# wpeebles/gangealing

Measured on NVIDIA H100. Metric: gangealing_train_images_per_sec_256, higher is better.
Workload: dtype f32

## Files before the change

### __graft_entry__.py

```python
import os
import sys

ROOT = os.path.dirname(os.path.abspath(__file__))
if ROOT not in sys.path:
    sys.path.insert(0, ROOT)


def build():
    from gangealing_b200 import build as gg_build
    lib = gg_build.build()
    from gangealing_b200 import _lib
    _lib.load()
    import gangealing_b200.op
    if os.path.isdir("/root/reference"):
        try:
            from oracle import build_ref
            build_ref.build()
        except Exception as exc:
            print("oracle/_ref not built: %s" % exc, file=sys.stderr)
    return lib


def smoke():
    import torch
# ... 37 lines not shown
          so.upfirdn2d_ref(x[:, :3], k, up=2, pad=(2, 1)), 1e-5)
    close("fused_leaky_relu", op.fused_leaky_relu(x.to(dev), b.to(dev)), so.fused_leaky_relu_ref(x, b), 1e-6)

    for dt, tol in ((torch.float32, 1e-4), (torch.bfloat16, 2e-2)):
        n, c = 2, 64
        raw = torch.randn(n, c, 17, 17, generator=g).to(dt).float()
        d, s_next = torch.rand(n, c, generator=g) + 0.5, torch.randn(n, c, generator=g) + 1
        nz = torch.randn(n, 1, 16, 16, generator=g)
        bb = torch.randn(c, generator=g)
        lo = [t.clone().requires_grad_(True) for t in (raw, d, s_next)]
        xs_o = so.blur_noise_bias_act_ref(lo[0], k, (1, 1), nz, nw, bb, row_scale=lo[1]) * lo[2][:, :, None, None]
        go = torch.randn(xs_o.shape, generator=g).to(dt).float()
        gr_o = torch.autograd.grad(xs_o, lo, go)
        lg = [raw.to(dev).to(dt).contiguous(memory_format=CL).requires_grad_(True), d.to(dev).requires_grad_(True),
              s_next.to(dev).requires_grad_(True)]
        xs, _ = fused_tail(lg[0], lg[1], lg[2], None, None, nz.to(dev), nw.to(dev), bb.to(dev), None, kernel=k.to(dev), pad=(1, 1))
        gr = torch.autograd.grad(xs, lg, go.to(dev).to(dt).contiguous(memory_format=CL))
        close("channels-last blur tail -> next conv input (%s)" % str(dt)[6:], xs, xs_o, tol)
        close("  its one-pass backward: d raw / d demod / d style (%s)" % str(dt)[6:], torch.cat([t.flatten().float().cpu() for t in gr]),
              torch.cat([t.flatten() for t in gr_o]), tol)
        raw2 = torch.randn(n, c, 16, 16, generator=g).to(dt).float()
        wm = torch.randn(n, 3, c, generator=g) / 8
        rb, skip = torch.randn(3, generator=g), torch.randn(n, 3, 16, 16, generator=g)
        o_ = so.noise_bias_act_ref(raw2 * d[:, :, None, None], nz, nw, bb)
        rgb_o = torch.einsum("noc,nchw->nohw", wm, o_) + rb.reshape(1, 3, 1, 1) + skip
        _, rgb = fused_tail(raw2.to(dev).to(dt).contiguous(memory_format=CL), d.to(dev), None, wm.to(dev), skip.to(dev), nz.to(dev),
                            nw.to(dev), bb.to(dev), rb.to(dev))
        close("channels-last conv tail + to-RGB in one pass (%s)" % str(dt)[6:], rgb, rgb_o, tol)

    w = [torch.randn(1, 128, 64, 3, 3, generator=g), torch.randn(1, 256, 128, 3, 3, generator=g)]
    st = [torch.randn(3, 64, generator=g), torch.randn(3, 128, generator=g)]
    dm = style_path.all_demod([t.to(dev) for t in w], [t.to(dev) for t in st], [0.04, 0.03])
    for wi, si, sc, di in zip(w, st, (0.04, 0.03), dm):
        want = torch.rsqrt(((sc * wi) * si.reshape(3, 1, -1, 1, 1)).pow(2).sum([2, 3, 4]) + 1e-8)
        close("wgmma demodulation GEMM (O=%d, I=%d)" % (wi.shape[1], wi.shape[2]), di, want, 1e-5)

    img = torch.rand(2, 3, 64, 64, generator=g) * 2 - 1
    theta = torch.tensor([[[0.7, 0.2, 0.05], [-0.2, 0.6, -0.1]], [[1.6, 0.0, 0.0], [0.0, 1.5, 0.1]]])
    out, grid, _ = S.stn_sample_affine(img.to(dev), theta.to(dev), (64, 64), 3.5, 0.0, "border")
    grid_o = osmp.affine_grid_ref(theta, (2, 3, 64, 64))
    close("one-pass similarity sampling: grid", grid, grid_o, 1e-5)
    close("one-pass similarity sampling: antialiased warp", out, osmp.mipmap_warp_ref(img, grid_o, 3.5, 0.0, "border"), 2e-3)
    low = 0.03 * torch.randn(2, 8, 8, 2, generator=g)
    mask = torch.randn(2, 576, 8, 8, generator=g)
    ident = osmp.affine_grid_ref(torch.eye(2, 3)[None], (1, 1, 64, 64))
    out, flow, delta, _ = S.stn_sample_flow(img.to(dev), low.to(dev), mask.to(dev), ident.to(dev), theta.to(dev), None, 8, 3.5, 0.0,
                                            "reflection")
    delta_o, flow_o = of.flow_compose_ref(low, mask, ident, theta, None, 8)
    close("one-pass flow sampling: composed flow", flow, flow_o, 1e-5)
    close("one-pass flow sampling: antialiased warp", out, osmp.mipmap_warp_ref(img, flow_o, 3.5, 0.0, "reflection"), 2e-3)
    close("BilinearDownsample (tent gather)", S.bilinear_downsample(img.to(dev), 2, *[t.to(dev) for t in _tent(3)]),
# ... 75 lines not shown
```

### gangealing_b200/_lib.py

```python
import ctypes
import os

import torch

_HERE = os.path.dirname(os.path.abspath(__file__))
LIB_PATH = os.path.join(_HERE, "libgg_b200.so")

GG_F32, GG_F16, GG_BF16 = 0, 1, 2
PAD_MODES = {"zeros": 0, "border": 1, "reflection": 2}

_c = ctypes
_P, _I, _L, _F = _c.c_void_p, _c.c_int, _c.c_int64, _c.c_float

SIGNATURES = {
    "gg_version": (_I, []),
    "gg_last_error": (_c.c_char_p, []),
    "gg_sm_count": (_I, []),
    "gg_fused_bias_act": (_I, [_P, _P, _P, _P, _I, _I, _I, _F, _F, _L, _L, _L, _P]),
    "gg_noise_bias_act": (_I, [_P, _P, _P, _P, _P, _P, _I, _F, _F, _L, _L, _L, _P]),
    "gg_channel_scale_workspace": (_L, [_L, _L]),
    "gg_channel_scale": (_I, [_P, _P, _P, _P, _P, _P, _I, _L, _L, _P]),
    "gg_bias_act_backward_workspace": (_L, [_L, _L, _L]),
    "gg_bias_act_backward": (_I, [_P, _P, _P, _P, _P, _I, _F, _F, _L, _L, _L, _P]),
    "gg_upfirdn2d": (_I, [_P, _P, _P, _I, _L] + [_I] * 12 + [_P]),
    "gg_blur_noise_bias_act": (_I, [_P] * 7 + [_I, _L, _L] + [_I] * 9 + [_F, _F, _P]),
    "gg_mipmap_pyramid_elems": (_L, [_L, _I, _I, _I]),
    "gg_mipmap_build": (_I, [_P, _P, _I, _L, _I, _I, _I, _P]),
    "gg_mipmap_build_backward": (_I, [_P, _P, _L, _I, _I, _I, _P]),
    "gg_mipmap_warp_forward": (_I, [_P] * 5 + [_I, _L] + [_I] * 6 + [_F, _F, _I, _P]),
    "gg_warp_sample_indices": (_I, [_P, _P, _L, _I, _I, _I, _I, _F, _F, _I, _P]),
    "gg_stn_sample_forward": (_I, [_P] * 11 + [_I, _I, _L] + [_I] * 9 + [_F, _F, _I, _P]),
    "gg_modconv_wsq": (_I, [_P, _P, _I, _I, _I, _P]),
    "gg_modconv_demod": (_I, [_P, _P, _P, _F, _F, _I, _I, _I, _P]),
    "gg_modconv_demod_batched": (_I, [_I, _P, _P, _P, _P, _P, _P, _F, _I, _P]),
    "gg_modconv_modulate": (_I, [_P, _P, _P, _P, _F, _I, _I, _I, _I, _I, _P]),
    "gg_noise_bias_act_nhwc": (_I, [_P] * 6 + [_I, _F, _F, _L, _I, _L, _P]),
    "gg_nhwc_rowwise_workspace": (_L, [_L, _I, _L]),
    "gg_channel_scale_nhwc": (_I, [_P] * 6 + [_I, _L, _I, _L, _P]),
    "gg_bias_act_backward_nhwc": (_I, [_P] * 5 + [_I, _F, _F, _L, _I, _L, _P]),
    "gg_blur_nhwc_workspace": (_L, [_I, _L] + [_I] * 9),
    "gg_blur_nhwc": (_I, [_P] * 12 + [_I, _L] + [_I] * 12 + [_F, _F, _P]),
    "gg_styled_tail_nhwc": (_I, [_P] * 12 + [_I, _I, _F, _F, _L, _I, _L, _P]),
    "gg_styled_tail_backward_workspace": (_L, [_I, _L, _I, _L]),
    "gg_styled_tail_backward_nhwc": (_I, [_P] * 12 + [_I, _F, _F, _L, _I, _L, _L, _P]),
    "gg_tent_downsample_forward": (_I, [_P] * 4 + [_L, _I, _I, _I, _I, _P]),
    "gg_tent_downsample_backward": (_I, [_P] * 4 + [_L, _I, _I, _I, _I, _P]),
    "gg_feature_distance_workspace": (_L, [_L, _I, _L]),
    "gg_feature_distance_forward": (_I, [_P] * 5 + [_I, _L, _I, _L, _F, _P]),
    "gg_feature_distance_backward": (_I, [_P] * 6 + [_I, _L, _I, _L, _F, _P]),
    "gg_bias_relu_pool_nhwc_forward": (_I, [_P, _P, _P, _P, _I, _L, _I, _I, _I, _P]),
    "gg_bias_relu_pool_nhwc_backward": (_I, [_P, _P, _P, _P, _I, _L, _I, _I, _I, _P]),
    "gg_to_rgb_nhwc_workspace": (_L, [_L, _I, _L]),
    "gg_to_rgb_nhwc_forward": (_I, [_P] * 5 + [_L, _I, _L, _P]),
    "gg_to_rgb_nhwc_backward": (_I, [_P] * 6 + [_L, _I, _L, _P]),
    "gg_nn_argmin_workspace": (_L, [_L, _L]),
    "gg_nn_argmin": (_I, [_P, _P, _P, _P, _L, _L, _I, _P]),
    "gg_splat2d_lookup_forward": (_I, [_P] * 8 + [_L, _L, _I, _I, _I, _I, _I, _F, _F, _I, _P]),
    "gg_scale_cast_multi": (_I, [_P, _P, _P, _I, _I, _P]),
    "gg_adam_ema_step": (_I, [_P, _P, _P, _I, _I, _P, _c.c_double, _c.c_double, _c.c_double, _c.c_double, _P]),
    "gg_tv_loss_workspace": (_L, [_L, _I, _I]),
    "gg_tv_loss_forward": (_I, [_P, _P, _P, _L, _I, _I, _P]),
    "gg_tv_loss_backward": (_I, [_P, _P, _P, _L, _I, _I, _P]),
    "gg_splat2d_workspace": (_L, [_L, _I, _I, _I]),
    "gg_splat2d_forward": (_I, [_P] * 6 + [_L, _L, _I, _I, _I, _I, _P]),
    "gg_flow_compose_forward": (_I, [_P] * 7 + [_L, _I, _I, _I, _P]),
    "gg_flow_compose_backward": (_I, [_P] * 10 + [_L, _I, _I, _I, _P]),
    "gg_mipmap_warp_backward": (_I, [_P] * 7 + [_I, _L] + [_I] * 6 + [_F, _F, _I, _P]),
# ... 143 lines not shown
```

### gangealing_b200/csrc/styled.cu

```cuda
#include "common.cuh"
#include "nhwc_reduce.cuh"

namespace gg {
namespace {

constexpr int kT = 256;
constexpr int kGroup = 8;
constexpr int kPix = 4;

struct TailFwdParams {
  const void* raw; void* out; void* xs; float* rgb; const float* skip;
  const float* noise; const float* noise_weight; const float* bias; const float* demod; const float* s_next;
  const float* wm; const float* rgb_bias;
  float alpha, gain;
  int act;
  int C;
  int64_t hw;
  int chunk, chunks_per_sample;
};

template <typename T, bool FAST>
__global__ void __launch_bounds__(kT, 2)
styled_tail_nhwc_kernel(const TailFwdParams p) {
  constexpr int V = ChanVec<T>::V;
  constexpr int Q = V / 4;
  extern __shared__ __align__(16) float cst[];
  const int C = p.C;
  const int nvec = C / V, J = nvec / kGroup;
  const int64_t n = blockIdx.x / p.chunks_per_sample;
  const int ck = blockIdx.x - n * p.chunks_per_sample;
  const int64_t p0 = static_cast<int64_t>(ck) * p.chunk, p1 = min(p0 + p.chunk, p.hw);
// ... 19 lines not shown
  const int l = threadIdx.x & (kGroup - 1), grp = threadIdx.x / kGroup;
  const unsigned gmask = 0xffu << (threadIdx.x & 24);
  const int hw = static_cast<int>(p.hw);
  const T* raw = static_cast<const T*>(p.raw) + n * hw * C;
  T* out = p.out ? static_cast<T*>(p.out) + n * hw * C : nullptr;
  T* xs = p.xs ? static_cast<T*>(p.xs) + n * hw * C : nullptr;
  const float* noise_n = p.noise ? p.noise + n * hw : nullptr;
  const int q0 = static_cast<int>(p0), q1 = static_cast<int>(p1);
  constexpr int kStride = (kT / kGroup) * kPix;
  auto pixel = [&](int pb_, int u) { return min(pb_ + u, q1 - 1); };
  uint4 xn[kPix];
  int pb = q0 + grp * kPix;
  if (pb < q1) {
#pragma unroll
    for (int u = 0; u < kPix; ++u) xn[u] = ldg_stream16(raw + static_cast<unsigned>(pixel(pb, u) * C + l * V));
  }
  for (; pb < q1; pb += kStride) {
    float nz[kPix];
    unsigned po[kPix];
#pragma unroll
    for (int u = 0; u < kPix; ++u) {
      const int px = pixel(pb, u);
      po[u] = static_cast<unsigned>(px) * static_cast<unsigned>(C);
      nz[u] = noise_n ? nw * __ldg(noise_n + px) : 0.f;
    }
    float acc[kPix][3];
#pragma unroll
    for (int u = 0; u < kPix; ++u) acc[u][0] = acc[u][1] = acc[u][2] = 0.f;
    for (int j = 0; j < J; ++j) {
      const int v = l + kGroup * j;
      uint4 xr[kPix];
#pragma unroll
      for (int u = 0; u < kPix; ++u) xr[u] = xn[u];
      {
        const bool wrap = (j + 1 == J);
        const int pbn = wrap ? pb + kStride : pb;
        const int vn = wrap ? l : v + kGroup;
        if (pbn < q1) {
#pragma unroll
          for (int u = 0; u < kPix; ++u) xn[u] = ldg_stream16(raw + static_cast<unsigned>(pixel(pbn, u) * C + vn * V));
        }
      }
      float d[V], b[V], s[V], w0[V], w1[V], w2[V];
#pragma unroll
      for (int q = 0; q < Q; ++q) {
        const float4 dv = c4[q * nvec + v], bv = c4[c4_plane + q * nvec + v], sv = c4[2 * c4_plane + q * nvec + v];
        d[4 * q] = dv.x; d[4 * q + 1] = dv.y; d[4 * q + 2] = dv.z; d[4 * q + 3] = dv.w;
        b[4 * q] = bv.x; b[4 * q + 1] = bv.y; b[4 * q + 2] = bv.z; b[4 * q + 3] = bv.w;
        s[4 * q] = sv.x; s[4 * q + 1] = sv.y; s[4 * q + 2] = sv.z; s[4 * q + 3] = sv.w;
        if (p.rgb) {
          const float4 a0 = c4[3 * c4_plane + q * nvec + v], a1 = c4[4 * c4_plane + q * nvec + v], a2 = c4[5 * c4_plane + q * nvec + v];
          w0[4 * q] = a0.x; w0[4 * q + 1] = a0.y; w0[4 * q + 2] = a0.z; w0[4 * q + 3] = a0.w;
          w1[4 * q] = a1.x; w1[4 * q + 1] = a1.y; w1[4 * q + 2] = a1.z; w1[4 * q + 3] = a1.w;
          w2[4 * q] = a2.x; w2[4 * q + 1] = a2.y; w2[4 * q + 2] = a2.z; w2[4 * q + 3] = a2.w;
        }
      }
#pragma unroll
      for (int u = 0; u < kPix; ++u) {
        float x[V], o[V], o2[V];
        ChanVec<T>::unpack(xr[u], x);
#pragma unroll
        for (int k = 0; k < V; ++k) {
          float t = fmaf(x[k], d[k], b[k] + nz[u]);
          t = fast ? fmaxf(t, t * neg) : (t > 0.f ? t : t * neg) * p.gain;
          o[k] = t;
          o2[k] = t * s[k];
        }
        if (p.rgb) {
#pragma unroll
          for (int k = 0; k < V; ++k) {
            acc[u][0] = fmaf(w0[k], o[k], acc[u][0]);
            acc[u][1] = fmaf(w1[k], o[k], acc[u][1]);
            acc[u][2] = fmaf(w2[k], o[k], acc[u][2]);
          }
        }
        if (pb + u < q1) {
          const unsigned off = po[u] + static_cast<unsigned>(v * V);
          if (out) stg_stream16(out + off, ChanVec<T>::pack(o));
          if (xs) stg_stream16(xs + off, ChanVec<T>::pack(o2));
        }
      }
    }
    if (p.rgb) {
#pragma unroll
      for (int m = kGroup / 2; m >= 1; m >>= 1)
#pragma unroll
        for (int u = 0; u < kPix; ++u)
#pragma unroll
          for (int o = 0; o < 3; ++o) acc[u][o] += __shfl_xor_sync(gmask, acc[u][o], m);
      if (l < 3) {
        const int o = l;
        const float rb = p.rgb_bias ? __ldg(p.rgb_bias + o) : 0.f;
        const int64_t off = (n * 3 + o) * p.hw + pb;
#pragma unroll
        for (int u = 0; u < kPix; ++u)
          if (pb + u < q1) {
            const float r = (o == 0 ? acc[u][0] : o == 1 ? acc[u][1] : acc[u][2]) + rb;
            p.rgb[off + u] = r + (p.skip ? __ldg(p.skip + off + u) : 0.f);
          }
      }
    }
  }
}

struct TailBwdParams {
  void* g_raw; float* partial;
  const void* g_xs; const void* out; const void* raw;
  const float* s_next; const float* demod; const float* g_rgb; const float* wm;
  float alpha, gain;
  int C;
  int64_t hw;
  int chunk, chunks_per_sample;
  int r_ds, r_dd, r_gw, n_red;
};

template <typename T>
__global__ void __launch_bounds__(kT, 2)
styled_tail_bwd_nhwc_kernel(const TailBwdParams p) {
  constexpr int V = ChanVec<T>::V;
  constexpr int U = (V == 4) ? 4 : 2;
  extern __shared__ float red[];
  const int C = p.C, cv = C / V;
  const int64_t n = blockIdx.x / p.chunks_per_sample;
  const int ck = blockIdx.x - n * p.chunks_per_sample;
  const int64_t p0 = static_cast<int64_t>(ck) * p.chunk, p1 = min(p0 + p.chunk, p.hw);
  const int lanes_p = kT / cv > 0 ? kT / cv : 1;
  const int cq = threadIdx.x % cv, pl = threadIdx.x / cv;
  float a_ds[V], a_dd[V], a_g0[V], a_g1[V], a_g2[V];
#pragma unroll
  for (int k = 0; k < V; ++k) a_ds[k] = a_dd[k] = a_g0[k] = a_g1[k] = a_g2[k] = 0.f;
  const T* gxs = static_cast<const T*>(p.g_xs);
  const T* outp = static_cast<const T*>(p.out);
  const T* rawp = static_cast<const T*>(p.raw);
  T* graw = static_cast<T*>(p.g_raw);
  if (pl < lanes_p) {
    float sv[V], dv[V], w0[V], w1[V], w2[V];
#pragma unroll
    for (int k = 0; k < V; ++k) {
      const int c = cq * V + k;
      sv[k] = p.s_next ? __ldg(p.s_next + n * C + c) : 1.f;
      dv[k] = p.demod ? __ldg(p.demod + n * C + c) : 1.f;
      w0[k] = p.g_rgb ? __ldg(p.wm + (n * 3 + 0) * C + c) : 0.f;
      w1[k] = p.g_rgb ? __ldg(p.wm + (n * 3 + 1) * C + c) : 0.f;
      w2[k] = p.g_rgb ? __ldg(p.wm + (n * 3 + 2) * C + c) : 0.f;
    }
    const float* g0 = p.g_rgb ? p.g_rgb + n * 3 * p.hw : nullptr;
    const uint4 zero = make_uint4(0u, 0u, 0u, 0u);
    auto body = [&](int64_t off, const uint4 gr, const uint4 orw, const uint4 rr, float s0, float s1, float s2) {
      float g[V], o[V], r[V], gt[V];
      ChanVec<T>::unpack(gr, g);
      ChanVec<T>::unpack(orw, o);
      ChanVec<T>::unpack(rr, r);
#pragma unroll
      for (int k = 0; k < V; ++k) {
        float go = g[k] * sv[k];
        if (p.g_rgb) go = fmaf(w2[k], s2, fmaf(w1[k], s1, fmaf(w0[k], s0, go)));
        const float t = (o[k] > 0.f ? go : go * p.alpha) * p.gain;
        a_ds[k] = fmaf(g[k], o[k], a_ds[k]);
        a_dd[k] = fmaf(t, r[k], a_dd[k]);
        a_g0[k] = fmaf(s0, o[k], a_g0[k]);
        a_g1[k] = fmaf(s1, o[k], a_g1[k]);
        a_g2[k] = fmaf(s2, o[k], a_g2[k]);
        gt[k] = t * dv[k];
      }
      *reinterpret_cast<uint4*>(graw + off) = ChanVec<T>::pack(gt);
    };
    int64_t pp = p0 + pl;
    for (; pp + (U - 1) * lanes_p < p1; pp += U * lanes_p) {
      uint4 gr[U], orw[U], rr[U];
      float s[U][3];
      int64_t off[U];
#pragma unroll
      for (int u = 0; u < U; ++u) {
        const int64_t pu = pp + u * lanes_p;
        off[u] = ((n * p.hw + pu) * cv + cq) * V;
        orw[u] = ldg_stream16(outp + off[u]);
        gr[u] = gxs ? ldg_stream16(gxs + off[u]) : zero;
      }
#pragma unroll
      for (int u = 0; u < U; ++u) {
        const int64_t pu = pp + u * lanes_p;
        rr[u] = rawp ? ldg_stream16(rawp + off[u]) : zero;
        s[u][0] = g0 ? __ldg(g0 + pu) : 0.f;
        s[u][1] = g0 ? __ldg(g0 + p.hw + pu) : 0.f;
        s[u][2] = g0 ? __ldg(g0 + 2 * p.hw + pu) : 0.f;
      }
#pragma unroll
      for (int u = 0; u < U; ++u) body(off[u], gr[u], orw[u], rr[u], s[u][0], s[u][1], s[u][2]);
    }
    for (; pp < p1; pp += lanes_p) {
      const int64_t off = ((n * p.hw + pp) * cv + cq) * V;
      body(off, gxs ? ldg_stream16(gxs + off) : zero, ldg_stream16(outp + off), rawp ? ldg_stream16(rawp + off) : zero,
           g0 ? __ldg(g0 + pp) : 0.f, g0 ? __ldg(g0 + p.hw + pp) : 0.f, g0 ? __ldg(g0 + 2 * p.hw + pp) : 0.f);
    }
  }
  if (p.partial && p.n_red > 0) {
    const int R = p.n_red;
    if (pl < lanes_p) {
      float* row = red + static_cast<int64_t>(pl) * R * C + cq * V;
#pragma unroll
      for (int k = 0; k < V; ++k) {
        if (p.r_ds >= 0) row[p.r_ds * C + k] = a_ds[k];
        if (p.r_dd >= 0) row[p.r_dd * C + k] = a_dd[k];
        if (p.r_gw >= 0) { row[p.r_gw * C + k] = a_g0[k]; row[(p.r_gw + 1) * C + k] = a_g1[k]; row[(p.r_gw + 2) * C + k] = a_g2[k]; }
      }
    }
    __syncthreads();
    for (int i = threadIdx.x; i < R * C; i += kT) {
      float t = 0.f;
      for (int q = 0; q < lanes_p; ++q) t += red[static_cast<int64_t>(q) * R * C + i];
      p.partial[static_cast<int64_t>(blockIdx.x) * R * C + i] = t;
    }
  }
}

// ... 50 lines not shown
  const size_t smem = static_cast<size_t>(6) * C * sizeof(float);
  auto st = static_cast<cudaStream_t>(stream);
  const bool fast = p.gain > 0.f && ((p.act == 3 && p.alpha >= 0.f && p.alpha <= 1.f) || p.act == 1);
  const unsigned g = static_cast<unsigned>(grid);
  if (dtype == GG_F32) {
    if (fast) styled_tail_nhwc_kernel<float, true><<<g, kT, smem, st>>>(p);
    else styled_tail_nhwc_kernel<float, false><<<g, kT, smem, st>>>(p);
  } else {
    if (fast) styled_tail_nhwc_kernel<__nv_bfloat16, true><<<g, kT, smem, st>>>(p);
    else styled_tail_nhwc_kernel<__nv_bfloat16, false><<<g, kT, smem, st>>>(p);
  }
  GG_CHECK_LAUNCH("styled_tail_nhwc launch");
  return GG_OK;
}

int64_t gg_styled_tail_backward_workspace(int dtype, int64_t N, int C, int64_t HW) {
  if (N <= 0 || C <= 0 || HW <= 0) return 0;
  const int V = dtype == GG_BF16 ? 8 : 4;
  if (C % V != 0) return 0;
  const int64_t chunk = bwd_chunk(N, C / V, HW);
  return N * ((HW + chunk - 1) / chunk) * 5 * C * static_cast<int64_t>(sizeof(float));
}

int gg_styled_tail_backward_nhwc(void* g_raw, float* d_s_next, float* d_demod, float* d_wm, void* workspace,
                                 const void* g_xs, const float* g_rgb, const void* out_saved, const void* raw,
                                 const float* s_next, const float* demod, const float* wm, int dtype, float alpha,
                                 float scale, int64_t N, int C, int64_t HW, int64_t reduce_pitch, void* stream) {
  if (N < 0 || C < 0 || HW < 0) return fail(GG_ERR_BAD_ARG, "styled_tail_backward_nhwc: negative size");
  if (dtype != GG_F32 && dtype != GG_BF16) return fail(GG_ERR_UNSUPPORTED, "styled_tail_backward_nhwc: dtype %d not supported", dtype);
  if (N * HW * C == 0) return GG_OK;
  const int V = dtype == GG_BF16 ? 8 : 4;
  if (C % V != 0 || C / V > kT) return fail(GG_ERR_UNSUPPORTED, "styled_tail_backward_nhwc: C must be a multiple of %d, <= %d", V, V * kT);
  if (!g_raw || !out_saved || (!g_xs && !g_rgb)) return fail(GG_ERR_BAD_ARG, "styled_tail_backward_nhwc: null tensor");
  if (g_xs && !s_next) return fail(GG_ERR_BAD_ARG, "styled_tail_backward_nhwc: g_xs needs s_next");
  if (g_rgb && !wm) return fail(GG_ERR_BAD_ARG, "styled_tail_backward_nhwc: g_rgb needs wm");
  if (d_s_next && !g_xs) return fail(GG_ERR_BAD_ARG, "styled_tail_backward_nhwc: d_s_next needs g_xs");
  if (d_demod && !raw) return fail(GG_ERR_BAD_ARG, "styled_tail_backward_nhwc: d_demod needs raw");
  if (d_wm && !g_rgb) return fail(GG_ERR_BAD_ARG, "styled_tail_backward_nhwc: d_wm needs g_rgb");
  if ((d_s_next || d_demod || d_wm) && !workspace) return fail(GG_ERR_BAD_ARG, "styled_tail_backward_nhwc: reductions need a workspace");
  const int cv = C / V;
  const int64_t chunk64 = bwd_chunk(N, cv, HW);
  if (chunk64 > 0x7fffffffLL) return fail(GG_ERR_BAD_ARG, "styled_tail_backward_nhwc: plane too large");
  const int K = static_cast<int>((HW + chunk64 - 1) / chunk64);
  const int64_t grid = N * K;
  if (grid > 0x7fffffffLL) return fail(GG_ERR_BAD_ARG, "styled_tail_backward_nhwc: too many CTAs");
  TailBwdParams p;
  p.g_raw = g_raw; p.partial = static_cast<float*>(workspace); p.g_xs = g_xs; p.out = out_saved;
  p.raw = d_demod ? raw : nullptr; p.s_next = s_next; p.demod = demod; p.g_rgb = g_rgb; p.wm = wm;
  p.alpha = alpha; p.gain = scale; p.C = C; p.hw = HW; p.chunk = static_cast<int>(chunk64); p.chunks_per_sample = K;
  int r = 0;
  p.r_ds = d_s_next ? r++ : -1;
  p.r_dd = d_demod ? r++ : -1;
  p.r_gw = d_wm ? r : -1;
  if (d_wm) r += 3;
  p.n_red = r;
  const int lanes_p = kT / cv > 0 ? kT / cv : 1;
  const size_t smem = static_cast<size_t>(lanes_p) * (r > 0 ? r : 1) * C * sizeof(float);
  auto st = static_cast<cudaStream_t>(stream);
  if (smem > 48 * 1024) {
    static DeviceOnce configured;
    if (configured.needed()) {
      cudaError_t e = cudaFuncSetAttribute(styled_tail_bwd_nhwc_kernel<float>, cudaFuncAttributeMaxDynamicSharedMemorySize, 100 * 1024);
      if (e == cudaSuccess)
        e = cudaFuncSetAttribute(styled_tail_bwd_nhwc_kernel<__nv_bfloat16>, cudaFuncAttributeMaxDynamicSharedMemorySize, 100 * 1024);
      if (e != cudaSuccess) return cuda_fail(e, "styled_tail_backward_nhwc smem opt-in");
      configured.done();
    }
    if (smem > 100 * 1024) return fail(GG_ERR_UNSUPPORTED, "styled_tail_backward_nhwc: C too large for the reduction stage");
  }
  if (dtype == GG_F32) styled_tail_bwd_nhwc_kernel<float><<<static_cast<unsigned>(grid), kT, smem, st>>>(p);
  else styled_tail_bwd_nhwc_kernel<__nv_bfloat16><<<static_cast<unsigned>(grid), kT, smem, st>>>(p);
  GG_CHECK_LAUNCH("styled_tail_backward_nhwc launch");
  if (r > 0) {
    float* first = d_s_next ? d_s_next : (d_demod ? d_demod : d_wm);
    const bool packed = (!d_s_next || d_s_next == first + static_cast<int64_t>(p.r_ds) * C) &&
                        (!d_demod || d_demod == first + static_cast<int64_t>(p.r_dd) * C) &&
                        (!d_wm || d_wm == first + static_cast<int64_t>(p.r_gw) * C) && reduce_pitch == r * C;
    if (packed) {
      nhwc_finish_kernel<<<static_cast<unsigned>(N * ((r * C + 31) / 32)), dim3(32, 32), 0, st>>>(
          first, static_cast<const float*>(workspace), N, K, r * C, r * C);
    } else {
      auto finish_row = [&](float* dst, int row, int rows_n) {
        nhwc_finish_kernel<<<static_cast<unsigned>(N * ((rows_n * C + 31) / 32)), dim3(32, 32), 0, st>>>(
            dst, static_cast<const float*>(workspace) + static_cast<int64_t>(row) * C, N, K, rows_n * C, r * C);
      };
      if (reduce_pitch != C && reduce_pitch != 0 && reduce_pitch != r * C)
        return fail(GG_ERR_BAD_ARG, "styled_tail_backward_nhwc: reduce_pitch must be C (separate dense outputs) or r*C (packed block)");
      if (d_s_next) finish_row(d_s_next, p.r_ds, 1);
      if (d_demod) finish_row(d_demod, p.r_dd, 1);
      if (d_wm) finish_row(d_wm, p.r_gw, 3);
    }
    GG_CHECK_LAUNCH("styled_tail_backward_nhwc finish launch");
  }
  return GG_OK;
}

}
```

### gangealing_b200/op/nhwc.py

```python
import torch

from .. import _lib

CL = torch.channels_last

TIMING = None


def elementwise_ok(t):
    return _lib.is_nhwc(t) and t.shape[1] % _lib.nhwc_vec(t) == 0


def rowwise_ok(t):
    return elementwise_ok(t) and t.shape[1] // _lib.nhwc_vec(t) <= 256


def blur_ok(t, kh, kw, up=(1, 1), down=(1, 1)):
    return (_lib.is_nhwc(t) and t.shape[1] % (8 * _lib.nhwc_vec(t)) == 0 and kh <= 4 and kw <= 4
            and up == (1, 1) and down == (1, 1))


def _f32(t, numel=None):
    if t is None:
        return None
# ... 99 lines not shown


def styled_tail(raw, noise, noise_weight, bias, demod, s_next, wm, rgb_bias, skip, want_out, negative_slope, gain, act=3):
    n, c, h, w = raw.shape
    out = torch.empty_like(raw) if want_out else None
    xs = torch.empty_like(raw) if s_next is not None else None
    rgb = torch.empty((n, 3, h, w), dtype=torch.float32, device=raw.device) if wm is not None else None
    sk = None
    if skip is not None and rgb is not None:
        sk = skip.detach()
        if sk.dtype != torch.float32 or not sk.is_contiguous():
            sk = sk.float().contiguous()
        if sk.shape != rgb.shape:
            raise RuntimeError("styled_tail: skip must be (N, 3, H, W)")
    rc = _lib.load().gg_styled_tail_nhwc(_lib.ptr(out), _lib.ptr(xs), _lib.ptr(rgb), raw.data_ptr(),
                                         _lib.ptr(noise_plane(noise, n, h, w)), _lib.ptr(_f32(noise_weight, 1)),
                                         _lib.ptr(_f32(bias, c)), _lib.ptr(_f32(demod, n * c)), _lib.ptr(_f32(s_next, n * c)),
                                         _lib.ptr(_f32(wm, n * 3 * c)), _lib.ptr(_f32(rgb_bias, 3)), _lib.ptr(sk),
                                         _lib.dtype_code(raw), act, negative_slope, gain, n, c, h * w, _lib.stream())
    _lib.check(rc, "gg_styled_tail_nhwc")
    return out, xs, rgb


def styled_tail_backward(g_xs, g_rgb, out_saved, raw, s_next, demod, wm, want_ds, want_dd, want_dwm, negative_slope, gain):
    n, c, h, w = out_saved.shape
    lib = _lib.load()
    dev = out_saved.device
    g_raw = torch.empty_like(out_saved)
    want_ds = want_ds and g_xs is not None
    want_dd = want_dd and raw is not None
    want_dwm = want_dwm and g_rgb is not None
    rows = int(want_ds) + int(want_dd) + 3 * int(want_dwm)
    block = torch.empty((n, rows, c), dtype=torch.float32, device=dev) if rows else None
    r = 0
    d_s = d_d = d_w = None
    if want_ds:
        d_s = block[:, r]; r += 1
    if want_dd:
        d_d = block[:, r]; r += 1
    if want_dwm:
        d_w = block[:, r:r + 3]
    code = _lib.dtype_code(out_saved)
    ws = None
    if rows:
        ws = torch.empty(max(1, lib.gg_styled_tail_backward_workspace(code, n, c, h * w) // 4), dtype=torch.float32, device=dev)
    rc = lib.gg_styled_tail_backward_nhwc(g_raw.data_ptr(), _lib.ptr(d_s), _lib.ptr(d_d), _lib.ptr(d_w), _lib.ptr(ws),
                                          _lib.ptr(g_xs), _lib.ptr(g_rgb), out_saved.data_ptr(),
                                          _lib.ptr(raw if want_dd else None),
                                          _lib.ptr(_f32(s_next, n * c)), _lib.ptr(_f32(demod, n * c)), _lib.ptr(_f32(wm, n * 3 * c)),
                                          code, negative_slope, gain, n, c, h * w, rows * c, _lib.stream())
    _lib.check(rc, "gg_styled_tail_backward_nhwc")
    return g_raw, d_s, d_d, d_w
```

### gangealing_b200/op/styled_fused.py

```python
import torch
from torch.autograd import Function
from torch.autograd.function import once_differentiable

from .. import _lib
from . import conv2d_gradfix, nhwc, style_path
from .modconv import channel_scale, shared_conv_weight
from .upfirdn2d import grad_pad, upfirdn2d

CL = torch.channels_last


class _FusedTail(Function):

    @staticmethod
    def forward(ctx, raw, demod, s_next, wm, skip, noise, noise_weight, bias, rgb_bias, kernel, pad, negative_slope, gain):
        _lib.require_cuda(raw, demod, s_next, wm, skip, noise)
        needs = ctx.needs_input_grad
        save = needs[0] or needs[1] or needs[2] or needs[3]
        if kernel is None:
            out, xs, rgb = nhwc.styled_tail(raw, noise, noise_weight, bias, demod, s_next, wm, rgb_bias, skip, save,
                                            negative_slope, gain)
        else:
            if wm is not None:
                raise RuntimeError("fused tail: the blur (up-sampling) layers carry no to-RGB branch")
            pad4 = (pad[0], pad[1], pad[0], pad[1])
            out, xs, _ = nhwc.blur(raw, kernel, pad4, mode=1, noise=noise, noise_weight=noise_weight, bias=bias,
                                   row_scale=demod, scale2=s_next, want_out=save or s_next is None,
                                   want_out2=s_next is not None, negative_slope=negative_slope, gain=gain)
            rgb = None
        ctx.cfg = (kernel is not None, pad, negative_slope, gain, tuple(raw.shape))
        if save:
            ctx.save_for_backward(raw if (needs[1] and demod is not None) else None, out,
                                  demod.detach() if demod is not None else None,
                                  s_next.detach() if s_next is not None else None,
                                  wm.detach() if wm is not None else None, kernel)
        if skip is not None and rgb is None:
            raise RuntimeError("fused tail: skip without a to-RGB branch")
        return xs, rgb

    @staticmethod
    @once_differentiable
    def backward(ctx, g_xs, g_rgb):
        raw, out, demod, s_next, wm, kernel = ctx.saved_tensors
        is_blur, pad, negative_slope, gain, raw_shape = ctx.cfg
        need_raw, need_d, need_s, need_w, need_skip = ctx.needs_input_grad[:5]
        if g_xs is not None:
            g_xs = g_xs.contiguous(memory_format=CL)
            if g_xs.dtype != out.dtype:
                g_xs = g_xs.to(out.dtype)
        if g_rgb is not None:
            g_rgb = g_rgb.float().contiguous()
        g_raw = d_s = d_d = d_w = None
        if g_xs is None and g_rgb is None:
            return (None,) * 13
        if not is_blur:
            g_raw, d_s, d_d, d_w = nhwc.styled_tail_backward(
                g_xs, g_rgb, out, raw, s_next, demod, wm, need_s, need_d and demod is not None, need_w,
                negative_slope, gain)
        else:
            g_t, d_s, _, _ = nhwc.styled_tail_backward(g_xs, None, out, None, s_next, None, None, need_s, False, False,
                                                       negative_slope, gain)
            kh, kw = kernel.shape
            pad4 = (pad[0], pad[1], pad[0], pad[1])
            gp = grad_pad(raw_shape[2], raw_shape[3], out.shape[2], out.shape[3], kh, kw, (1, 1), (1, 1), pad4)
            want_dot = need_d and demod is not None
            g_raw, _, d_d = nhwc.blur(g_t, _lib.flipped_filter(kernel), gp, mode=2, row_scale=demod, mul=raw if want_dot else None,
                                      want_dot=want_dot)
            if tuple(g_raw.shape) != raw_shape:
                raise RuntimeError("fused tail backward: adjoint produced %s, expected %s" % (tuple(g_raw.shape), raw_shape))
        return (g_raw if need_raw else None, d_d if need_d else None, d_s if need_s else None, d_w if need_w else None,
                g_rgb if need_skip else None, None, None, None, None, None, None, None, None)


def fused_tail(raw, demod, s_next, wm, skip, noise, noise_weight, bias, rgb_bias, kernel=None, pad=None, negative_slope=0.2,
               gain=2 ** 0.5):
    return _FusedTail.apply(raw, demod, s_next, wm, skip, noise, noise_weight, bias, rgb_bias, kernel, pad, negative_slope, gain)


def fusable(generator, latent, act_dtype):
    if not latent.is_cuda or getattr(generator, "num_fp16_res", 0) != 0 and not generator.run_fp32:
        return False
# ... 58 lines not shown
```

### include/gg_b200.h

```cpp
#ifndef GG_B200_H_
#define GG_B200_H_

#include <stdint.h>

#ifdef __cplusplus
extern "C" {
#endif

#define GG_API __attribute__((visibility("default")))

enum { GG_F32 = 0, GG_F16 = 1, GG_BF16 = 2, GG_F64 = 3 };

enum {
  GG_OK = 0,
  GG_ERR_BAD_ARG = -1,
  GG_ERR_UNSUPPORTED = -2,
  GG_ERR_CUDA = -3
};

enum { GG_PAD_ZEROS = 0, GG_PAD_BORDER = 1, GG_PAD_REFLECTION = 2 };

GG_API int gg_version(void);
GG_API const char* gg_last_error(void);
GG_API int gg_sm_count(void);
// ... 78 lines not shown
GG_API int gg_channel_scale_nhwc(void* out, float* row_dot, void* workspace, const void* x, const void* y,
                                 const float* s, int dtype, int64_t N, int C, int64_t HW, void* stream);
GG_API int gg_bias_act_backward_nhwc(void* gx, float* grad_bias, void* workspace, const void* g,
                                     const void* out_saved, int dtype, float alpha, float scale, int64_t N, int C,
                                     int64_t HW, void* stream);
GG_API int64_t gg_blur_nhwc_workspace(int dtype, int64_t N, int C, int in_h, int in_w, int kernel_h, int kernel_w,
                                      int pad_x0, int pad_x1, int pad_y0, int pad_y1);
GG_API int gg_blur_nhwc(void* out, void* out2, const void* in, const float* kernel, const float* noise,
                        const float* noise_weight, const float* bias, const float* row_scale, const float* scale2,
                        const void* mul, float* row_dot, void* workspace, int dtype, int64_t N, int C, int in_h,
                        int in_w, int kernel_h, int kernel_w, int separable, int pad_x0, int pad_x1, int pad_y0,
                        int pad_y1, int mode, int act, float alpha, float scale, void* stream);

GG_API int gg_styled_tail_nhwc(void* out, void* xs, float* rgb, const void* raw, const float* noise,
                               const float* noise_weight, const float* bias, const float* demod, const float* s_next,
                               const float* wm, const float* rgb_bias, const float* skip, int dtype, int act,
                               float alpha, float scale, int64_t N, int C, int64_t HW, void* stream);
GG_API int64_t gg_styled_tail_backward_workspace(int dtype, int64_t N, int C, int64_t HW);
GG_API int gg_styled_tail_backward_nhwc(void* g_raw, float* d_s_next, float* d_demod, float* d_wm, void* workspace,
                                        const void* g_xs, const float* g_rgb, const void* out_saved, const void* raw,
                                        const float* s_next, const float* demod, const float* wm, int dtype,
                                        float alpha, float scale, int64_t N, int C, int64_t HW, int64_t reduce_pitch,
                                        void* stream);

GG_API int64_t gg_to_rgb_nhwc_workspace(int64_t N, int C, int64_t HW);
GG_API int gg_to_rgb_nhwc_forward(float* out, const float* x, const float* wm, const float* bias, const float* skip,
                                  int64_t N, int C, int64_t HW, void* stream);
GG_API int gg_to_rgb_nhwc_backward(float* gx, float* gwm, void* workspace, const float* g, const float* x,
                                   const float* wm, int64_t N, int C, int64_t HW, void* stream);


GG_API int64_t gg_feature_distance_workspace(int64_t N, int C, int64_t HW);
GG_API int gg_feature_distance_forward(float* out, void* workspace, const void* f0, const void* f1,
                                       const float* weight, int dtype, int64_t N, int C, int64_t HW, float eps,
                                       void* stream);
GG_API int gg_feature_distance_backward(void* g0, void* g1, const float* grad_out, const void* f0, const void* f1,
                                        const float* weight, int dtype, int64_t N, int C, int64_t HW, float eps,
                                        void* stream);

GG_API int gg_bias_relu_pool_nhwc_forward(void* y, void* pooled, const void* raw, const float* bias, int dtype, int64_t N,
                                          int C, int H, int W, void* stream);
GG_API int gg_bias_relu_pool_nhwc_backward(void* grad_raw, const void* grad_y, const void* grad_pooled, const void* y,
                                           int dtype, int64_t N, int C, int H, int W, void* stream);

GG_API int gg_tent_downsample_forward(float* out, const float* in, const float* taps_h, const float* taps_v, int64_t N,
                                      int C, int in_h, int in_w, int stride, void* stream);
// ... 45 lines not shown
```

Measured before the change: 376.0.

## Recompute styled-tail activation in backward instead of saving output

The non-blur styled tail forward no longer writes the activation output. The backward kernel instead recomputes it from the raw conv result using demod, bias and noise, with the per-channel folded constants staged in shared memory. This removes one full activation write in forward and one read in backward, at the cost of extra arithmetic and noise loads in the backward pass. The backward now needs noise, noise weight and bias kept alive, and uses a smaller unroll for bf16.

```diff
diff --git a/__graft_entry__.py b/__graft_entry__.py
--- a/__graft_entry__.py
+++ b/__graft_entry__.py
@@ -83,11 +83,18 @@
         raw2 = torch.randn(n, c, 16, 16, generator=g).to(dt).float()
         wm = torch.randn(n, 3, c, generator=g) / 8
         rb, skip = torch.randn(3, generator=g), torch.randn(n, 3, 16, 16, generator=g)
-        o_ = so.noise_bias_act_ref(raw2 * d[:, :, None, None], nz, nw, bb)
-        rgb_o = torch.einsum("noc,nchw->nohw", wm, o_) + rb.reshape(1, 3, 1, 1) + skip
-        _, rgb = fused_tail(raw2.to(dev).to(dt).contiguous(memory_format=CL), d.to(dev), None, wm.to(dev), skip.to(dev), nz.to(dev),
-                            nw.to(dev), bb.to(dev), rb.to(dev))
+        lo = [t.clone().requires_grad_(True) for t in (raw2, d, wm)]
+        o_ = so.noise_bias_act_ref(lo[0] * lo[1][:, :, None, None], nz, nw, bb)
+        rgb_o = torch.einsum("noc,nchw->nohw", lo[2], o_) + rb.reshape(1, 3, 1, 1) + skip
+        g_rgb = torch.randn(rgb_o.shape, generator=g)
+        gr_o = torch.autograd.grad(rgb_o, lo, g_rgb)
+        lg = [raw2.to(dev).to(dt).contiguous(memory_format=CL).requires_grad_(True), d.to(dev).requires_grad_(True),
+              wm.to(dev).requires_grad_(True)]
+        _, rgb = fused_tail(lg[0], lg[1], None, lg[2], skip.to(dev), nz.to(dev), nw.to(dev), bb.to(dev), rb.to(dev))
         close("channels-last conv tail + to-RGB in one pass (%s)" % str(dt)[6:], rgb, rgb_o, tol)
+        gr = torch.autograd.grad(rgb, lg, g_rgb.to(dev))
+        close("  its backward, activation recomputed from raw: d raw / d demod / d wm (%s)" % str(dt)[6:],
+              torch.cat([t.flatten().float().cpu() for t in gr]), torch.cat([t.flatten() for t in gr_o]), tol)
 
     w = [torch.randn(1, 128, 64, 3, 3, generator=g), torch.randn(1, 256, 128, 3, 3, generator=g)]
     st = [torch.randn(3, 64, generator=g), torch.randn(3, 128, generator=g)]
diff --git a/gangealing_b200/_lib.py b/gangealing_b200/_lib.py
--- a/gangealing_b200/_lib.py
+++ b/gangealing_b200/_lib.py
@@ -43,6 +43,7 @@
     "gg_styled_tail_nhwc": (_I, [_P] * 12 + [_I, _I, _F, _F, _L, _I, _L, _P]),
     "gg_styled_tail_backward_workspace": (_L, [_I, _L, _I, _L]),
     "gg_styled_tail_backward_nhwc": (_I, [_P] * 12 + [_I, _F, _F, _L, _I, _L, _L, _P]),
+    "gg_styled_tail_backward_recompute_nhwc": (_I, [_P] * 14 + [_I, _I, _F, _F, _L, _I, _L, _L, _P]),
     "gg_tent_downsample_forward": (_I, [_P] * 4 + [_L, _I, _I, _I, _I, _P]),
     "gg_tent_downsample_backward": (_I, [_P] * 4 + [_L, _I, _I, _I, _I, _P]),
     "gg_feature_distance_workspace": (_L, [_L, _I, _L]),
diff --git a/gangealing_b200/csrc/styled.cu b/gangealing_b200/csrc/styled.cu
--- a/gangealing_b200/csrc/styled.cu
+++ b/gangealing_b200/csrc/styled.cu
@@ -7,6 +7,13 @@
 constexpr int kT = 256;
 constexpr int kGroup = 8;
 constexpr int kPix = 4;
+
+template <bool FAST>
+__device__ __forceinline__ float tail_act(float x, float d, float b, float nz, float neg, float gain) {
+  const float t = __fmaf_rn(x, d, __fadd_rn(b, nz));
+  const float tn = __fmul_rn(t, neg);
+  return FAST ? fmaxf(t, tn) : __fmul_rn(t > 0.f ? t : tn, gain);
+}
 
 struct TailFwdParams {
   const void* raw; void* out; void* xs; float* rgb; const float* skip;
@@ -72,7 +79,7 @@
     for (int u = 0; u < kPix; ++u) {
       const int px = pixel(pb, u);
       po[u] = static_cast<unsigned>(px) * static_cast<unsigned>(C);
-      nz[u] = noise_n ? nw * __ldg(noise_n + px) : 0.f;
+      nz[u] = noise_n ? __fmul_rn(nw, __ldg(noise_n + px)) : 0.f;
     }
     float acc[kPix][3];
 #pragma unroll
@@ -111,10 +118,8 @@
         ChanVec<T>::unpack(xr[u], x);
 #pragma unroll
         for (int k = 0; k < V; ++k) {
-          float t = fmaf(x[k], d[k], b[k] + nz[u]);
-          t = fast ? fmaxf(t, t * neg) : (t > 0.f ? t : t * neg) * p.gain;
-          o[k] = t;
-          o2[k] = t * s[k];
+          o[k] = tail_act<FAST>(x[k], d[k], b[k], nz[u], neg, p.gain);
+          o2[k] = o[k] * s[k];
         }
         if (p.rgb) {
 #pragma unroll
@@ -157,25 +162,36 @@
   void* g_raw; float* partial;
   const void* g_xs; const void* out; const void* raw;
   const float* s_next; const float* demod; const float* g_rgb; const float* wm;
+  const float* noise; const float* noise_weight; const float* bias;
   float alpha, gain;
+  int act;
   int C;
   int64_t hw;
   int chunk, chunks_per_sample;
   int r_ds, r_dd, r_gw, n_red;
 };
 
-template <typename T>
+template <typename T, bool RECOMPUTE, bool FAST>
 __global__ void __launch_bounds__(kT, 2)
 styled_tail_bwd_nhwc_kernel(const TailBwdParams p) {
   constexpr int V = ChanVec<T>::V;
-  constexpr int U = (V == 4) ? 4 : 2;
-  extern __shared__ float red[];
+  constexpr int U = (V == 4) ? 4 : (RECOMPUTE ? 1 : 2);
+  extern __shared__ __align__(16) float smem_f[];
+  float* red = smem_f + (RECOMPUTE ? 2 * p.C : 0);
   const int C = p.C, cv = C / V;
   const int64_t n = blockIdx.x / p.chunks_per_sample;
   const int ck = blockIdx.x - n * p.chunks_per_sample;
   const int64_t p0 = static_cast<int64_t>(ck) * p.chunk, p1 = min(p0 + p.chunk, p.hw);
   const int lanes_p = kT / cv > 0 ? kT / cv : 1;
   const int cq = threadIdx.x % cv, pl = threadIdx.x / cv;
+  const float gfold = FAST ? p.gain : 1.f;
+  if constexpr (RECOMPUTE) {
+    for (int c = threadIdx.x; c < C; c += kT) {
+      smem_f[c] = (p.demod ? __ldg(p.demod + n * C + c) : 1.f) * gfold;
+      smem_f[C + c] = (p.bias ? __ldg(p.bias + c) : 0.f) * gfold;
+    }
+    __syncthreads();
+  }
   float a_ds[V], a_dd[V], a_g0[V], a_g1[V], a_g2[V];
 #pragma unroll
   for (int k = 0; k < V; ++k) a_ds[k] = a_dd[k] = a_g0[k] = a_g1[k] = a_g2[k] = 0.f;
@@ -184,6 +200,7 @@
   const T* rawp = static_cast<const T*>(p.raw);
   T* graw = static_cast<T*>(p.g_raw);
   if (pl < lanes_p) {
+    const float neg = (p.act == 3) ? p.alpha : 1.f;
     float sv[V], dv[V], w0[V], w1[V], w2[V];
 #pragma unroll
     for (int k = 0; k < V; ++k) {
@@ -194,13 +211,31 @@
       w1[k] = p.g_rgb ? __ldg(p.wm + (n * 3 + 1) * C + c) : 0.f;
       w2[k] = p.g_rgb ? __ldg(p.wm + (n * 3 + 2) * C + c) : 0.f;
     }
+    const float4* dfold4 = reinterpret_cast<const float4*>(smem_f) + cq * (V / 4);
+    const float4* bfold4 = reinterpret_cast<const float4*>(smem_f + C) + cq * (V / 4);
+    const float nw = RECOMPUTE ? (p.noise ? (p.noise_weight ? __ldg(p.noise_weight) : 1.f) : 0.f) * gfold : 0.f;
+    const float* noise_n = (RECOMPUTE && p.noise) ? p.noise + n * p.hw : nullptr;
+    auto noise_at = [&](int64_t pu) { return noise_n ? __fmul_rn(nw, __ldg(noise_n + pu)) : 0.f; };
     const float* g0 = p.g_rgb ? p.g_rgb + n * 3 * p.hw : nullptr;
     const uint4 zero = make_uint4(0u, 0u, 0u, 0u);
-    auto body = [&](int64_t off, const uint4 gr, const uint4 orw, const uint4 rr, float s0, float s1, float s2) {
+    auto body = [&](int64_t off, const uint4 gr, const uint4 orw, const uint4 rr, float nz, float s0, float s1, float s2) {
       float g[V], o[V], r[V], gt[V];
       ChanVec<T>::unpack(gr, g);
-      ChanVec<T>::unpack(orw, o);
-      ChanVec<T>::unpack(rr, r);
+      if constexpr (RECOMPUTE) {
+        ChanVec<T>::unpack(orw, r);
+#pragma unroll
+        for (int q = 0; q < V / 4; ++q) {
+          const float4 d4 = dfold4[q], b4 = bfold4[q];
+          o[4 * q + 0] = tail_act<FAST>(r[4 * q + 0], d4.x, b4.x, nz, neg, p.gain);
+          o[4 * q + 1] = tail_act<FAST>(r[4 * q + 1], d4.y, b4.y, nz, neg, p.gain);
+          o[4 * q + 2] = tail_act<FAST>(r[4 * q + 2], d4.z, b4.z, nz, neg, p.gain);
+          o[4 * q + 3] = tail_act<FAST>(r[4 * q + 3], d4.w, b4.w, nz, neg, p.gain);
+        }
+        ChanVec<T>::unpack(ChanVec<T>::pack(o), o);
+      } else {
+        ChanVec<T>::unpack(orw, o);
+        ChanVec<T>::unpack(rr, r);
+      }
 #pragma unroll
       for (int k = 0; k < V; ++k) {
         float go = g[k] * sv[k];
@@ -216,31 +251,34 @@
       *reinterpret_cast<uint4*>(graw + off) = ChanVec<T>::pack(gt);
     };
     int64_t pp = p0 + pl;
+    const T* orwp = RECOMPUTE ? rawp : outp;
     for (; pp + (U - 1) * lanes_p < p1; pp += U * lanes_p) {
       uint4 gr[U], orw[U], rr[U];
-      float s[U][3];
+      float s[U][3], nz[U];
       int64_t off[U];
 #pragma unroll
       for (int u = 0; u < U; ++u) {
         const int64_t pu = pp + u * lanes_p;
         off[u] = ((n * p.hw + pu) * cv + cq) * V;
-        orw[u] = ldg_stream16(outp + off[u]);
+        orw[u] = ldg_stream16(orwp + off[u]);
         gr[u] = gxs ? ldg_stream16(gxs + off[u]) : zero;
       }
 #pragma unroll
       for (int u = 0; u < U; ++u) {
         const int64_t pu = pp + u * lanes_p;
-        rr[u] = rawp ? ldg_stream16(rawp + off[u]) : zero;
+        rr[u] = (!RECOMPUTE && rawp) ? ldg_stream16(rawp + off[u]) : zero;
+        nz[u] = noise_at(pu);
         s[u][0] = g0 ? __ldg(g0 + pu) : 0.f;
         s[u][1] = g0 ? __ldg(g0 + p.hw + pu) : 0.f;
         s[u][2] = g0 ? __ldg(g0 + 2 * p.hw + pu) : 0.f;
       }
 #pragma unroll
-      for (int u = 0; u < U; ++u) body(off[u], gr[u], orw[u], rr[u], s[u][0], s[u][1], s[u][2]);
+      for (int u = 0; u < U; ++u) body(off[u], gr[u], orw[u], rr[u], nz[u], s[u][0], s[u][1], s[u][2]);
     }
     for (; pp < p1; pp += lanes_p) {
       const int64_t off = ((n * p.hw + pp) * cv + cq) * V;
-      body(off, gxs ? ldg_stream16(gxs + off) : zero, ldg_stream16(outp + off), rawp ? ldg_stream16(rawp + off) : zero,
+      body(off, gxs ? ldg_stream16(gxs + off) : zero, ldg_stream16(orwp + off),
+           (!RECOMPUTE && rawp) ? ldg_stream16(rawp + off) : zero, noise_at(pp),
            g0 ? __ldg(g0 + pp) : 0.f, g0 ? __ldg(g0 + p.hw + pp) : 0.f, g0 ? __ldg(g0 + 2 * p.hw + pp) : 0.f);
     }
   }
@@ -337,16 +375,21 @@
   return N * ((HW + chunk - 1) / chunk) * 5 * C * static_cast<int64_t>(sizeof(float));
 }
 
-int gg_styled_tail_backward_nhwc(void* g_raw, float* d_s_next, float* d_demod, float* d_wm, void* workspace,
-                                 const void* g_xs, const float* g_rgb, const void* out_saved, const void* raw,
-                                 const float* s_next, const float* demod, const float* wm, int dtype, float alpha,
-                                 float scale, int64_t N, int C, int64_t HW, int64_t reduce_pitch, void* stream) {
+}
+
+static int launch_tail_backward(void* g_raw, float* d_s_next, float* d_demod, float* d_wm, void* workspace,
+                                const void* g_xs, const float* g_rgb, const void* out_saved, const void* raw,
+                                const float* noise, const float* noise_weight, const float* bias, const float* s_next,
+                                const float* demod, const float* wm, int dtype, int act, float alpha, float scale,
+                                int64_t N, int C, int64_t HW, int64_t reduce_pitch, void* stream) {
+  const bool recompute = out_saved == nullptr;
   if (N < 0 || C < 0 || HW < 0) return fail(GG_ERR_BAD_ARG, "styled_tail_backward_nhwc: negative size");
   if (dtype != GG_F32 && dtype != GG_BF16) return fail(GG_ERR_UNSUPPORTED, "styled_tail_backward_nhwc: dtype %d not supported", dtype);
+  if (act != 1 && act != 3) return fail(GG_ERR_UNSUPPORTED, "styled_tail_backward_nhwc: act must be 1 (linear) or 3 (lrelu)");
   if (N * HW * C == 0) return GG_OK;
   const int V = dtype == GG_BF16 ? 8 : 4;
   if (C % V != 0 || C / V > kT) return fail(GG_ERR_UNSUPPORTED, "styled_tail_backward_nhwc: C must be a multiple of %d, <= %d", V, V * kT);
-  if (!g_raw || !out_saved || (!g_xs && !g_rgb)) return fail(GG_ERR_BAD_ARG, "styled_tail_backward_nhwc: null tensor");
+  if (!g_raw || (recompute && !raw) || (!g_xs && !g_rgb)) return fail(GG_ERR_BAD_ARG, "styled_tail_backward_nhwc: null tensor");
   if (g_xs && !s_next) return fail(GG_ERR_BAD_ARG, "styled_tail_backward_nhwc: g_xs needs s_next");
   if (g_rgb && !wm) return fail(GG_ERR_BAD_ARG, "styled_tail_backward_nhwc: g_rgb needs wm");
   if (d_s_next && !g_xs) return fail(GG_ERR_BAD_ARG, "styled_tail_backward_nhwc: d_s_next needs g_xs");
@@ -361,7 +404,8 @@
   if (grid > 0x7fffffffLL) return fail(GG_ERR_BAD_ARG, "styled_tail_backward_nhwc: too many CTAs");
   TailBwdParams p;
   p.g_raw = g_raw; p.partial = static_cast<float*>(workspace); p.g_xs = g_xs; p.out = out_saved;
-  p.raw = d_demod ? raw : nullptr; p.s_next = s_next; p.demod = demod; p.g_rgb = g_rgb; p.wm = wm;
+  p.raw = (recompute || d_demod) ? raw : nullptr; p.s_next = s_next; p.demod = demod; p.g_rgb = g_rgb; p.wm = wm;
+  p.noise = noise; p.noise_weight = noise_weight; p.bias = bias; p.act = act;
   p.alpha = alpha; p.gain = scale; p.C = C; p.hw = HW; p.chunk = static_cast<int>(chunk64); p.chunks_per_sample = K;
   int r = 0;
   p.r_ds = d_s_next ? r++ : -1;
@@ -370,21 +414,36 @@
   if (d_wm) r += 3;
   p.n_red = r;
   const int lanes_p = kT / cv > 0 ? kT / cv : 1;
-  const size_t smem = static_cast<size_t>(lanes_p) * (r > 0 ? r : 1) * C * sizeof(float);
+  const size_t smem = (static_cast<size_t>(lanes_p) * (r > 0 ? r : 1) + (recompute ? 2 : 0)) * C * sizeof(float);
   auto st = static_cast<cudaStream_t>(stream);
   if (smem > 48 * 1024) {
     static DeviceOnce configured;
     if (configured.needed()) {
-      cudaError_t e = cudaFuncSetAttribute(styled_tail_bwd_nhwc_kernel<float>, cudaFuncAttributeMaxDynamicSharedMemorySize, 100 * 1024);
-      if (e == cudaSuccess)
-        e = cudaFuncSetAttribute(styled_tail_bwd_nhwc_kernel<__nv_bfloat16>, cudaFuncAttributeMaxDynamicSharedMemorySize, 100 * 1024);
+      const void* kernels[6] = {reinterpret_cast<const void*>(styled_tail_bwd_nhwc_kernel<float, false, false>),
+                                reinterpret_cast<const void*>(styled_tail_bwd_nhwc_kernel<float, true, false>),
+                                reinterpret_cast<const void*>(styled_tail_bwd_nhwc_kernel<float, true, true>),
+                                reinterpret_cast<const void*>(styled_tail_bwd_nhwc_kernel<__nv_bfloat16, false, false>),
+                                reinterpret_cast<const void*>(styled_tail_bwd_nhwc_kernel<__nv_bfloat16, true, false>),
+                                reinterpret_cast<const void*>(styled_tail_bwd_nhwc_kernel<__nv_bfloat16, true, true>)};
+      cudaError_t e = cudaSuccess;
+      for (int i = 0; i < 6 && e == cudaSuccess; ++i)
+        e = cudaFuncSetAttribute(kernels[i], cudaFuncAttributeMaxDynamicSharedMemorySize, 100 * 1024);
       if (e != cudaSuccess) return cuda_fail(e, "styled_tail_backward_nhwc smem opt-in");
       configured.done();
     }
     if (smem > 100 * 1024) return fail(GG_ERR_UNSUPPORTED, "styled_tail_backward_nhwc: C too large for the reduction stage");
   }
-  if (dtype == GG_F32) styled_tail_bwd_nhwc_kernel<float><<<static_cast<unsigned>(grid), kT, smem, st>>>(p);
-  else styled_tail_bwd_nhwc_kernel<__nv_bfloat16><<<static_cast<unsigned>(grid), kT, smem, st>>>(p);
+  const bool fast = scale > 0.f && ((act == 3 && alpha >= 0.f && alpha <= 1.f) || act == 1);
+  const unsigned g = static_cast<unsigned>(grid);
+  if (dtype == GG_F32) {
+    if (!recompute) styled_tail_bwd_nhwc_kernel<float, false, false><<<g, kT, smem, st>>>(p);
+    else if (fast) styled_tail_bwd_nhwc_kernel<float, true, true><<<g, kT, smem, st>>>(p);
+    else styled_tail_bwd_nhwc_kernel<float, true, false><<<g, kT, smem, st>>>(p);
+  } else {
+    if (!recompute) styled_tail_bwd_nhwc_kernel<__nv_bfloat16, false, false><<<g, kT, smem, st>>>(p);
+    else if (fast) styled_tail_bwd_nhwc_kernel<__nv_bfloat16, true, true><<<g, kT, smem, st>>>(p);
+    else styled_tail_bwd_nhwc_kernel<__nv_bfloat16, true, false><<<g, kT, smem, st>>>(p);
+  }
   GG_CHECK_LAUNCH("styled_tail_backward_nhwc launch");
   if (r > 0) {
     float* first = d_s_next ? d_s_next : (d_demod ? d_demod : d_wm);
@@ -410,4 +469,24 @@
   return GG_OK;
 }
 
-}
+extern "C" {
+
+int gg_styled_tail_backward_nhwc(void* g_raw, float* d_s_next, float* d_demod, float* d_wm, void* workspace,
+                                 const void* g_xs, const float* g_rgb, const void* out_saved, const void* raw,
+                                 const float* s_next, const float* demod, const float* wm, int dtype, float alpha,
+                                 float scale, int64_t N, int C, int64_t HW, int64_t reduce_pitch, void* stream) {
+  if (!out_saved && N * HW * C != 0) return fail(GG_ERR_BAD_ARG, "styled_tail_backward_nhwc: null saved output");
+  return launch_tail_backward(g_raw, d_s_next, d_demod, d_wm, workspace, g_xs, g_rgb, out_saved, raw, nullptr, nullptr,
+                              nullptr, s_next, demod, wm, dtype, 3, alpha, scale, N, C, HW, reduce_pitch, stream);
+}
+
+int gg_styled_tail_backward_recompute_nhwc(void* g_raw, float* d_s_next, float* d_demod, float* d_wm, void* workspace,
+                                           const void* g_xs, const float* g_rgb, const void* raw, const float* noise,
+                                           const float* noise_weight, const float* bias, const float* s_next,
+                                           const float* demod, const float* wm, int dtype, int act, float alpha,
+                                           float scale, int64_t N, int C, int64_t HW, int64_t reduce_pitch, void* stream) {
+  return launch_tail_backward(g_raw, d_s_next, d_demod, d_wm, workspace, g_xs, g_rgb, nullptr, raw, noise, noise_weight,
+                              bias, s_next, demod, wm, dtype, act, alpha, scale, N, C, HW, reduce_pitch, stream);
+}
+
+}
diff --git a/gangealing_b200/op/nhwc.py b/gangealing_b200/op/nhwc.py
--- a/gangealing_b200/op/nhwc.py
+++ b/gangealing_b200/op/nhwc.py
@@ -145,11 +145,14 @@
     return out, xs, rgb
 
 
-def styled_tail_backward(g_xs, g_rgb, out_saved, raw, s_next, demod, wm, want_ds, want_dd, want_dwm, negative_slope, gain):
-    n, c, h, w = out_saved.shape
+def styled_tail_backward(g_xs, g_rgb, out_saved, raw, s_next, demod, wm, want_ds, want_dd, want_dwm, negative_slope, gain,
+                         noise=None, noise_weight=None, bias=None, act=3):
+    recompute = out_saved is None
+    like = raw if recompute else out_saved
+    n, c, h, w = like.shape
     lib = _lib.load()
-    dev = out_saved.device
-    g_raw = torch.empty_like(out_saved)
+    dev = like.device
+    g_raw = torch.empty_like(like)
     want_ds = want_ds and g_xs is not None
     want_dd = want_dd and raw is not None
     want_dwm = want_dwm and g_rgb is not None
@@ -163,14 +166,19 @@
         d_d = block[:, r]; r += 1
     if want_dwm:
         d_w = block[:, r:r + 3]
-    code = _lib.dtype_code(out_saved)
+    code = _lib.dtype_code(like)
     ws = None
     if rows:
         ws = torch.empty(max(1, lib.gg_styled_tail_backward_workspace(code, n, c, h * w) // 4), dtype=torch.float32, device=dev)
-    rc = lib.gg_styled_tail_backward_nhwc(g_raw.data_ptr(), _lib.ptr(d_s), _lib.ptr(d_d), _lib.ptr(d_w), _lib.ptr(ws),
-                                          _lib.ptr(g_xs), _lib.ptr(g_rgb), out_saved.data_ptr(),
-                                          _lib.ptr(raw if want_dd else None),
-                                          _lib.ptr(_f32(s_next, n * c)), _lib.ptr(_f32(demod, n * c)), _lib.ptr(_f32(wm, n * 3 * c)),
-                                          code, negative_slope, gain, n, c, h * w, rows * c, _lib.stream())
-    _lib.check(rc, "gg_styled_tail_backward_nhwc")
+    sums = (g_raw.data_ptr(), _lib.ptr(d_s), _lib.ptr(d_d), _lib.ptr(d_w), _lib.ptr(ws), _lib.ptr(g_xs), _lib.ptr(g_rgb))
+    consts = (_lib.ptr(_f32(s_next, n * c)), _lib.ptr(_f32(demod, n * c)), _lib.ptr(_f32(wm, n * 3 * c)))
+    if recompute:
+        rc = lib.gg_styled_tail_backward_recompute_nhwc(*sums, raw.data_ptr(), _lib.ptr(noise_plane(noise, n, h, w)),
+                                                        _lib.ptr(_f32(noise_weight, 1)), _lib.ptr(_f32(bias, c)), *consts,
+                                                        code, act, negative_slope, gain, n, c, h * w, rows * c, _lib.stream())
+        _lib.check(rc, "gg_styled_tail_backward_recompute_nhwc")
+    else:
+        rc = lib.gg_styled_tail_backward_nhwc(*sums, out_saved.data_ptr(), _lib.ptr(raw if want_dd else None), *consts,
+                                              code, negative_slope, gain, n, c, h * w, rows * c, _lib.stream())
+        _lib.check(rc, "gg_styled_tail_backward_nhwc")
     return g_raw, d_s, d_d, d_w
diff --git a/gangealing_b200/op/styled_fused.py b/gangealing_b200/op/styled_fused.py
--- a/gangealing_b200/op/styled_fused.py
+++ b/gangealing_b200/op/styled_fused.py
@@ -18,7 +18,7 @@
         needs = ctx.needs_input_grad
         save = needs[0] or needs[1] or needs[2] or needs[3]
         if kernel is None:
-            out, xs, rgb = nhwc.styled_tail(raw, noise, noise_weight, bias, demod, s_next, wm, rgb_bias, skip, save,
+            out, xs, rgb = nhwc.styled_tail(raw, noise, noise_weight, bias, demod, s_next, wm, rgb_bias, skip, False,
                                             negative_slope, gain)
         else:
             if wm is not None:
@@ -30,10 +30,12 @@
             rgb = None
         ctx.cfg = (kernel is not None, pad, negative_slope, gain, tuple(raw.shape))
         if save:
-            ctx.save_for_backward(raw if (needs[1] and demod is not None) else None, out,
+            recompute = kernel is None
+            ctx.save_for_backward(raw if (recompute or (needs[1] and demod is not None)) else None, out,
                                   demod.detach() if demod is not None else None,
                                   s_next.detach() if s_next is not None else None,
-                                  wm.detach() if wm is not None else None, kernel)
+                                  wm.detach() if wm is not None else None, kernel,
+                                  *((noise, noise_weight, bias) if recompute else (None, None, None)))
         if skip is not None and rgb is None:
             raise RuntimeError("fused tail: skip without a to-RGB branch")
         return xs, rgb
@@ -41,13 +43,14 @@
     @staticmethod
     @once_differentiable
     def backward(ctx, g_xs, g_rgb):
-        raw, out, demod, s_next, wm, kernel = ctx.saved_tensors
+        raw, out, demod, s_next, wm, kernel, noise, noise_weight, bias = ctx.saved_tensors
         is_blur, pad, negative_slope, gain, raw_shape = ctx.cfg
         need_raw, need_d, need_s, need_w, need_skip = ctx.needs_input_grad[:5]
+        act_dtype = out.dtype if is_blur else raw.dtype
         if g_xs is not None:
             g_xs = g_xs.contiguous(memory_format=CL)
-            if g_xs.dtype != out.dtype:
-                g_xs = g_xs.to(out.dtype)
+            if g_xs.dtype != act_dtype:
+                g_xs = g_xs.to(act_dtype)
         if g_rgb is not None:
             g_rgb = g_rgb.float().contiguous()
         g_raw = d_s = d_d = d_w = None
@@ -55,8 +58,8 @@
             return (None,) * 13
         if not is_blur:
             g_raw, d_s, d_d, d_w = nhwc.styled_tail_backward(
-                g_xs, g_rgb, out, raw, s_next, demod, wm, need_s, need_d and demod is not None, need_w,
-                negative_slope, gain)
+                g_xs, g_rgb, None, raw, s_next, demod, wm, need_s, need_d and demod is not None, need_w,
+                negative_slope, gain, noise=noise, noise_weight=noise_weight, bias=bias)
         else:
             g_t, d_s, _, _ = nhwc.styled_tail_backward(g_xs, None, out, None, s_next, None, None, need_s, False, False,
                                                        negative_slope, gain)
diff --git a/include/gg_b200.h b/include/gg_b200.h
--- a/include/gg_b200.h
+++ b/include/gg_b200.h
@@ -124,6 +124,12 @@
                                         const float* s_next, const float* demod, const float* wm, int dtype,
                                         float alpha, float scale, int64_t N, int C, int64_t HW, int64_t reduce_pitch,
                                         void* stream);
+GG_API int gg_styled_tail_backward_recompute_nhwc(void* g_raw, float* d_s_next, float* d_demod, float* d_wm,
+                                                  void* workspace, const void* g_xs, const float* g_rgb, const void* raw,
+                                                  const float* noise, const float* noise_weight, const float* bias,
+                                                  const float* s_next, const float* demod, const float* wm, int dtype,
+                                                  int act, float alpha, float scale, int64_t N, int C, int64_t HW,
+                                                  int64_t reduce_pitch, void* stream);
 
 GG_API int64_t gg_to_rgb_nhwc_workspace(int64_t N, int C, int64_t HW);
 GG_API int gg_to_rgb_nhwc_forward(float* out, const float* x, const float* wm, const float* bias, const float* skip,
```

Measured after the change: 383.6, median of 6. 1.02x the previous value.
